# TCGGroup/Torch_Detection

Hardware: AMD Instinct MI355X
Metric: images/sec ResNet-50-FPN fwd+bwd 1333x800 (higher is better)
Workload: dtype bf16; 1 GPU; ResNet-50 + FPN(256, 5 levels) forward+backward, 2 x 3x800x1344 (1333x800 zero-padded to /32) per GPU, BN eval (reference default), fixed cotangents, all parameter grads; global_batch=2, parallelism=dp1, weights_static=True

## Files before the change

### include/tdn.h

```cpp
#ifndef TDN_H_
#define TDN_H_

#include <stddef.h>
#include <stdint.h>

#ifdef __cplusplus
extern "C" {
#endif

#define TDN_VERSION 100

enum { TDN_BF16 = 0, TDN_F16 = 1 };

enum {
  TDN_ADD_NONE = 0,
  TDN_ADD_SAME = 1,
  TDN_ADD_UP2X = 2,
  TDN_ADD_SUMPOOL2 = 3
};

typedef struct tdn_epilogue {
  const float* scale;
  const float* shift;
  const void* addend;
// ... 30 lines not shown

int64_t tdn_conv2d_wgrad_workspace(int N, int H, int W, int Cin, int Cout, int k, int stride,
                                    int pad);

int tdn_conv2d_wgrad(const void* x, const void* g, const void* w_fwd, const float* scale,
                     const float* mean, const float* invstd, float* dw, float* dgamma,
                     float* dbeta, float beta, int N, int H, int W, int Cin, int Cout, int k,
                     int stride, int pad, void* workspace, int64_t workspace_bytes, int dtype,
                     void* stream);

enum { TDN_WGRAD_CONV = 0, TDN_WGRAD_STEM = 1, TDN_WGRAD_GCONV = 2 };
typedef struct tdn_wgrad_item {
  const void* x;
  const void* g;
  const void* w_fwd;
  const float* scale;
  const float* mean;
  const float* invstd;
  float* dw;
  float* dgamma;
  float* dbeta;
  float beta;
  int32_t kind;
  int32_t N, H, W;
  int32_t Cin, Cout;
  int32_t k, stride, pad;
  int32_t groups;
  int32_t reserved;
} tdn_wgrad_item;
int64_t tdn_wgrad_group_workspace(const tdn_wgrad_item* items, int n, int dtype);
int tdn_wgrad_group(const tdn_wgrad_item* items, int n, void* workspace, int64_t workspace_bytes, int dtype,
                    void* stream);
int tdn_wgrad_group_plan(const tdn_wgrad_item* items, int n, int dtype, int32_t* per_item, int32_t* totals);

typedef struct tdn_prep_item {
  const float* w;
  void* w_fwd;
  void* w_dgrad;
  const float* gamma;
  const float* beta;
  const float* mean;
  const float* var;
  float* fold;
  int64_t s_o, s_i, s_h, s_w;
  int32_t Cout, Cin, kh, kw;
  float eps;
  int32_t reserved;
} tdn_prep_item;
int tdn_prepare_group(const tdn_prep_item* items, int n, int dtype, void* stream);

typedef struct tdn_bottleneck_args {
  const void* in;
  const void* w1;
  const void* w2;
  const void* w3;
  const float* scale1; const float* shift1;
  const float* scale2; const float* shift2;
  const float* scale3; const float* shift3;
  const void* mask1;
  const void* mask2;
  const void* mask3;
  void* out1;
  void* out2;
  void* out3;
  int32_t N, H, W, C;
  void* bits1;
// ... 300 lines not shown
```

### torch_detection_amd/_lib.py

```python
import ctypes
import os
import threading

import torch

_HERE = os.path.dirname(os.path.abspath(__file__))
LIB_PATH = os.path.join(_HERE, os.path.basename(os.environ.get("TDN_LIB", "") or "libtdn.so"))

TDN_BF16 = 0
TDN_F16 = 1
TDN_F32 = 2
NMS_SEG_MAX = 4096
RPN_MAX_LEVELS = 8
RPN_MAX_NUM = 8192
ROI_MAX_LEVELS = 8
ROI_MAX_OUT = 16
ROI_MAX_SAMPLES = 512
TARGET_MAX_GT = 256
TARGET_MAX_BOXES = 1 << 20
TARGET_MAX_NUM = 8192
LOSS_MAX_LEVELS = 8
LOSS_MAX_CLASSES = 1024
LOSS_MAX_ROWS = 1 << 20
LOSS_MAX_AVG = 64
# ... 132 lines not shown
                ("scale3", c_void_p), ("shift3", c_void_p),
                ("mask1", c_void_p), ("mask2", c_void_p), ("mask3", c_void_p),
                ("out1", c_void_p), ("out2", c_void_p), ("out3", c_void_p),
                ("N", ctypes.c_int32), ("H", ctypes.c_int32), ("W", ctypes.c_int32), ("C", ctypes.c_int32),
                ("bits1", c_void_p), ("bits2", c_void_p), ("bits3", c_void_p)]


_BA = ctypes.POINTER(BottleneckArgs)


class BottleneckHeadArgs(ctypes.Structure):
    _fields_ = [("b", BottleneckArgs), ("addend", c_void_p), ("wd", c_void_p), ("scale_d", c_void_p),
                ("shift_d", c_void_p)]


_BHA = ctypes.POINTER(BottleneckHeadArgs)

SIGNATURES = {
    "tdn_last_error": (ctypes.c_char_p, []),
    "tdn_version": (c_int, []),
    "tdn_bn_fold": (c_int, [c_void_p] * 4 + [c_float, c_int] + [c_void_p] * 3 + [c_void_p]),
    "tdn_pack_conv_weight": (c_int, [c_void_p, c_i64, c_i64, c_i64, c_i64, c_int, c_int, c_int, c_int,
                                     c_void_p, c_void_p, c_void_p, c_int, c_void_p]),
    "tdn_pack_stem_weight": (c_int, [c_void_p, c_int, c_void_p, c_int, c_void_p]),
    "tdn_prepare_group": (c_int, [_PI, c_int, c_int, c_void_p]),
    "tdn_conv2d_fwd": (c_int, [c_void_p] * 3 + [c_int] * 8 + [_EP, c_int, c_void_p]),
    "tdn_conv2d_dgrad": (c_int, [c_void_p] * 3 + [c_int] * 8 + [_EP, c_int, c_void_p]),
    "tdn_conv2d_wgrad_workspace": (c_i64, [c_int] * 8),
    "tdn_conv2d_wgrad": (c_int, [c_void_p] * 9 + [c_float] + [c_int] * 8 + [c_void_p, c_i64, c_int, c_void_p]),
    "tdn_wgrad_group_workspace": (c_i64, [_WI, c_int, c_int]),
    "tdn_wgrad_group": (c_int, [_WI, c_int, c_void_p, c_i64, c_int, c_void_p]),
    "tdn_wgrad_group_plan": (c_int, [_WI, c_int, c_int, ctypes.POINTER(ctypes.c_int32),
                                     ctypes.POINTER(ctypes.c_int32)]),
    "tdn_stage_image": (c_int, [c_void_p, c_i64, c_i64, c_i64, c_i64, c_int, c_int, c_int, c_void_p, c_int,
                                c_void_p]),
    "tdn_stem_conv_fwd": (c_int, [c_void_p] * 3 + [c_int] * 4 + [_EP, c_int, c_void_p]),
    "tdn_stem_pool_fwd": (c_int, [c_void_p] * 6 + [c_int] * 5 + [c_void_p]),
    "tdn_stem_conv_wgrad_workspace": (c_i64, [c_int] * 4),
    "tdn_stem_conv_wgrad": (c_int, [c_void_p] * 9 + [c_float] + [c_int] * 4 + [c_void_p, c_i64, c_int, c_void_p]),
    "tdn_maxpool3x3s2_fwd": (c_int, [c_void_p] * 3 + [c_int] * 5 + [c_void_p]),
    "tdn_maxpool3x3s2_bwd": (c_int, [c_void_p] * 4 + [c_int] * 5 + [c_void_p]),
    "tdn_maxpool3x3s2_relu_bwd": (c_int, [c_void_p] * 4 + [c_int] * 5 + [c_void_p]),
    "tdn_subsample2_fwd": (c_int, [c_void_p] * 2 + [c_int] * 5 + [c_void_p]),
    "tdn_subsample2_bwd": (c_int, [c_void_p] * 3 + [c_int] * 5 + [c_void_p]),
    "tdn_add_relu_mask": (c_int, [c_void_p] * 4 + [c_i64, c_int, c_void_p]),
    "tdn_clamp_max": (c_int, [c_void_p, c_float, c_i64, c_int, c_void_p]),
    "tdn_act_mask": (c_int, [c_void_p] * 3 + [c_float, c_i64, c_int, c_void_p]),
    "tdn_channel_affine_fwd": (c_int, [c_void_p] * 4 + [c_i64, c_int, c_int, c_int, c_void_p]),
    "tdn_channel_affine_bwd_workspace": (c_i64, [c_i64, c_int]),
    "tdn_channel_affine_bwd": (c_int, [c_void_p] * 8 + [c_float, c_i64, c_int, c_void_p, c_i64, c_int, c_void_p]),
    "tdn_nchw_f32_to_nhwc": (c_int, [c_void_p, c_i64, c_i64, c_i64, c_i64, c_int, c_int, c_int, c_int, c_void_p,
                                     c_int, c_void_p]),
    "tdn_nchw16_to_nhwc": (c_int, [c_void_p, c_i64, c_i64, c_i64, c_i64, c_int, c_int, c_int, c_int, c_void_p,
                                   c_void_p]),
    "tdn_nhwc_to_nchw_f32": (c_int, [c_void_p, c_int, c_int, c_int, c_int, c_void_p, c_int, c_void_p]),
    "tdn_anchor_grid": (c_int, [c_void_p, c_int, c_int, c_int, c_int, c_int, c_int, c_void_p, c_void_p, c_void_p]),
    "tdn_anchor_pyramid": (c_int, [_AL, c_int, c_void_p, c_void_p, c_void_p]),
    "tdn_bbox_iou_pairwise": (c_int, [c_void_p, c_int, c_void_p, c_int, c_void_p, c_void_p]),
    "tdn_nms_workspace": (c_i64, [c_int]),
    "tdn_nms": (c_int, [c_void_p, c_void_p, c_int, c_float, c_void_p, c_void_p, c_void_p, c_void_p, c_i64,
                        c_void_p]),
    "tdn_bbox_normalize": (c_int, [c_void_p, c_i64, ctypes.POINTER(c_float), ctypes.POINTER(c_float), c_void_p]),
    "tdn_bbox_denormalize": (c_int, [c_void_p, c_void_p, c_i64, c_int, ctypes.POINTER(c_float),
                                     ctypes.POINTER(c_float), c_void_p]),
    "tdn_bbox2delta": (c_int, [c_void_p, c_void_p, c_i64, ctypes.POINTER(c_float), ctypes.POINTER(c_float), c_void_p,
                               c_void_p]),
# ... 123 lines not shown
```

### torch_detection_amd/csrc/conv_wgrad.hip

```cpp
#include "conv_host.h"
#include <limits.h>
#include <string.h>
#include <type_traits>
#include <algorithm>
#include <math.h>
#include <mutex>
#include <unordered_map>
#include <vector>

constexpr int WG_MAXI = 26;
constexpr int FIN_MAXI = 30;

struct WgItem {
  const bf16_t* x;
  const bf16_t* g;
  const bf16_t* w_fwd;
  const float* scale;
  float* out;
  float* colsum;
  float* dotpart;
  int Hin, Win, Cpix, Ktap;
  int Ho, Wo, Cout, sa;
  int M, Mchunk, splitk;
  int ntaps, Ktot;
  int tiles_co, tiles_k;
  int tapgen;
  int grouped;
  int direct;
  float beta;
  int reserved;
};

struct WgGroup {
  int nitems, reserved;
  int blk_start[WG_MAXI + 2];
  WgItem it[WG_MAXI];
};
static_assert(sizeof(WgGroup) <= 4096, "kernel-argument block too large");

__device__ __forceinline__ void wg_tap(int tapgen, int t, int& dh, int& dw) {
  const int k = tapgen & 0xff, pad = (tapgen >> 8) & 0xff, dil = (tapgen >> 16) & 0xff;
  if (tapgen >> 24) { dh = t; dw = 0; return; }
  const int kh = t / k, kw = t - kh * k;
  dh = kh * dil - pad;
  dw = kw * dil - pad;
}

__device__ __forceinline__ bool wg_work(int bid, int splitk, int ntiles, int& split, int& tile) {
  if (splitk >= 8) {
    const int xj = bid >> 3;
    split = (bid & 7) + 8 * (xj / ntiles);
    tile = xj - (xj / ntiles) * ntiles;
  } else {
    split = bid / ntiles;
    tile = bid - split * ntiles;
  }
  return split < splitk;
}
static int wg_blocks(int splitk, int ntiles) {
  const int slots = splitk >= 8 ? 8 * ((splitk + 7) / 8) : splitk;
  return (slots * ntiles + 7) & ~7;
}

template <int RB>
__device__ __forceinline__ int tr_swz(int row) {
  if constexpr (RB >= 256) return (row & 3) | (((row >> 3) & 1) << 2);
  else if constexpr (RB == 128) return ((row >> 1) & 1) | (((row >> 3) & 1) << 1);
  else return (row >> 3) & 1;
}

template <int N>
__device__ __forceinline__ void wg_wait_vm_and_barrier() {
  asm volatile("s_waitcnt vmcnt(%0)\n\ts_barrier" ::"n"(N) : "memory");
}

#ifdef TDN_TRACE_BUILD
__device__ unsigned long long* g_wg_trace = nullptr;
__device__ int g_wg_trace_cap = 0;
#define WG_STAMP(slot, val)                                                                        \
  do {                                                                                             \
    if (g_wg_trace && tid == 0 && (int)blockIdx.x < g_wg_trace_cap)                                \
      g_wg_trace[(size_t)blockIdx.x * 8 + (slot)] = (unsigned long long)(val);                     \
  } while (0)
extern "C" int tdn_debug_wgrad_trace(void* buf, int nwg_cap) {
  unsigned long long* b = (unsigned long long*)buf;
  hipError_t e = hipMemcpyToSymbol(HIP_SYMBOL(g_wg_trace), &b, sizeof(b));
  TDN_CHECK(e == hipSuccess, "tdn_debug_wgrad_trace: %s", hipGetErrorString(e));
  e = hipMemcpyToSymbol(HIP_SYMBOL(g_wg_trace_cap), &nwg_cap, sizeof(nwg_cap));
  TDN_CHECK(e == hipSuccess, "tdn_debug_wgrad_trace: %s", hipGetErrorString(e));
  return 0;
}
#else
#define WG_STAMP(slot, val) do { } while (0)
#endif

template <int BMW , int BNW , int WM, int WN, int NST, bool F16>
__global__ __launch_bounds__(WM * WN * 64) void conv_wgrad_group_kernel(const WgGroup grp) {
  extern __shared__ __attribute__((aligned(16))) char smem[];
  constexpr int BKW = 64;
  constexpr int RBG = BMW * 2, RBX = BNW * 2;
  constexpr int G_BYTES = BKW * RBG, X_BYTES = BKW * RBX, STAGE = G_BYTES + X_BYTES;
  constexpr int RPIG = 1024 / RBG, RPIX = 1024 / RBX;
  constexpr int NW = WM * WN;
  constexpr int G_IT = BKW / (RPIG * NW), X_IT = BKW / (RPIX * NW);
  static_assert(G_IT >= 1 && X_IT >= 1, "every wave must issue the same number of loads per stage (counted vmcnt)");
  constexpr int LOADS = G_IT + X_IT;
  static_assert(LOADS * (NST - 2) < 64, "vmcnt immediate out of range");
  constexpr int WTM = BMW / WM, WTN = BNW / WN, FM = WTM / 16, FN = WTN / 16;
  static_assert(FM >= 1 && FN >= 1, "tile too small");
  static_assert((RPIG * NW) % 16 == 0 && (RPIX * NW) % 16 == 0, "loader round must be a multiple of 16 rows");
  static_assert(WN * BMW * 4 <= NST * STAGE, "cross-wave reduction buffer must fit the ring");

  const int tid = threadIdx.x;
  const int lane = tid & 63;
  const int wave = __builtin_amdgcn_readfirstlane(tid >> 6);

  int idx = 0;
#pragma unroll
  for (int i = 1; i < WG_MAXI; ++i) idx += ((int)blockIdx.x >= grp.blk_start[i]) ? 1 : 0;
  const WgItem& p = grp.it[idx];
  const int ntiles = p.tiles_co * p.tiles_k;
  int split, tile;
  if (!wg_work((int)blockIdx.x - grp.blk_start[idx], p.splitk, ntiles, split, tile)) return;
  WG_STAMP(0, __builtin_readcyclecounter());
  WG_STAMP(4, __builtin_amdgcn_s_memrealtime());
  const int tile_co = tile % p.tiles_co, tile_k = tile / p.tiles_co;
  const int co0 = tile_co * BMW;
  const int kt_per_tap = p.Ktap / BNW;
  const int tap_i = tile_k / kt_per_tap;
  const int ci_k = (tile_k - tap_i * kt_per_tap) * BNW;
  const int ci0 = p.grouped ? co0 : ci_k;
  int dh, dw;
  wg_tap(p.tapgen, tap_i, dh, dw);
  const int m_begin = split * p.Mchunk;
  const int m_end = min(p.M, m_begin + p.Mchunk);
  const int Cout = p.Cout, Cpix = p.Cpix, Hin = p.Hin, Win = p.Win, sa = p.sa, Wo = p.Wo, Ho = p.Ho;
  const bf16_t* const gx = p.x;
  const bf16_t* const gg = p.g;

  constexpr int CPRG = RBG / 16, CPRX = RBX / 16;
  const int g_lrow = lane / CPRG, g_pc = lane % CPRG;
  const int x_lrow = lane / CPRX, x_pc = lane % CPRX;
  const int g_row0 = wave * RPIG + g_lrow;
  const int x_row0 = wave * RPIX + x_lrow;
  const int g_src_el = ((((g_pc >> 1) ^ tr_swz<RBG>(g_row0)) << 1) | (g_pc & 1)) * 8;
  const int x_src_el = ((((x_pc >> 1) ^ tr_swz<RBX>(x_row0)) << 1) | (x_pc & 1)) * 8;
  const bf16_t* zero = (const bf16_t*)g_zero_page;

  int xa[X_IT], xb[X_IT], ximg[X_IT];
  const int HoWo = Ho * Wo;
#pragma unroll
  for (int it = 0; it < X_IT; ++it) {
    const int m = m_begin + it * (RPIX * NW) + x_row0;
    const int img = m / HoWo;
    const int rem = m - img * HoWo;
    ximg[it] = img;
// ... 157 lines not shown
      float d = dpart[i];
      d += __shfl_xor(d, 16, 64);
      d += __shfl_xor(d, 32, 64);
      if (grp4 == 0) red[wn * BMW + wm * WTM + i * 16 + fr] = d;
    }
    __syncthreads();
    for (int c = tid; c < BMW; c += NW * 64) {
      float s = red[c];
#pragma unroll
      for (int w = 1; w < WN; ++w) s += red[w * BMW + c];
      p.dotpart[(int64_t)tile_k * Cout + co0 + c] = s;
    }
  }
}

template <bool F16, int WMR = 4>
__global__ __launch_bounds__(WMR * 128) void conv_wgrad9_group_kernel(const WgGroup grp) {
  extern __shared__ __attribute__((aligned(16))) char smem[];
  constexpr int BKW = 64, BMW = 32 * WMR, BNW = 64;
  constexpr int NWV = WMR * 2;
  constexpr int RBG = BMW * 2, RBX = BNW * 2;
  constexpr int CPRG = RBG / 16, RPIG = 64 / CPRG;
  constexpr int XIT = 64 / (NWV * 8);
  static_assert(RPIG * NWV == 32 && XIT >= 1, "loader layout");
  constexpr int G_TILE = BKW * RBG;
  constexpr int XROWS = 72;
  constexpr int X_TILE = XROWS * RBX;
  constexpr int STAGE = G_TILE + 3 * X_TILE;
  constexpr int FM = 2, FN = 2, WN = 2, WTM = 16 * FM, WTN = 16 * FN;
  const int tid = threadIdx.x;
  const int lane = tid & 63;
  const int wave = __builtin_amdgcn_readfirstlane(tid >> 6);

  int idx = 0;
#pragma unroll
  for (int i = 1; i < WG_MAXI; ++i) idx += ((int)blockIdx.x >= grp.blk_start[i]) ? 1 : 0;
  const WgItem& p = grp.it[idx];
  const int ntiles = p.tiles_co * p.tiles_k;
  int split, tile;
  if (!wg_work((int)blockIdx.x - grp.blk_start[idx], p.splitk, ntiles, split, tile)) return;
  const int tile_co = tile % p.tiles_co, tile_ci = tile / p.tiles_co;
  const int co0 = tile_co * BMW, ci0 = tile_ci * BNW;
  const int m_begin = split * p.Mchunk;
  const int pM = p.M;
  const int m_end = min(pM, m_begin + p.Mchunk);
  const int W = p.Wo, H = p.Ho;
  const int Cout = p.Cout, Cpix = p.Cpix;
  const bf16_t* const gx = p.x;
  const bf16_t* const gg = p.g;
  const bf16_t* zero = (const bf16_t*)g_zero_page;

  const int g_lrow = lane / CPRG, g_pc = lane % CPRG;
  const int x_lrow = lane >> 3, x_pc = lane & 7;
  const int g_row0 = wave * RPIG + g_lrow;
  const int x_row0 = wave * 8 + x_lrow;
  const int g_src_el = ((((g_pc >> 1) ^ tr_swz<RBG>(g_row0)) << 1) | (g_pc & 1)) * 8;
  const int x_src_el = ((((x_pc >> 1) ^ tr_swz<RBX>(x_row0)) << 1) | (x_pc & 1)) * 8;
  int xh[XIT + 1], xw[XIT + 1];
#pragma unroll
  for (int it = 0; it <= XIT; ++it) {
    const int q = m_begin + it * (NWV * 8) + x_row0 - 1;
    const int qq = q < 0 ? q + W * H : q;
    xw[it] = qq % W;
    xh[it] = (qq / W) % H;
  }

  auto stage_load = [&](int mt, int s) {
    char* sG = smem + s * STAGE;
    char* sX = sG + G_TILE;
#pragma unroll
    for (int it = 0; it < 2; ++it) {
      const int m = mt + it * 32 + g_row0;
      const bf16_t* src = (m < m_end) ? gg + ((int64_t)m * Cout + co0 + g_src_el) : zero + (g_src_el & 127);
// ... 329 lines not shown
    if (tid == 0) {
      const float d = (red[0] + red[1]) + (red[2] + red[3]);
      if (p.dbeta) p.dbeta[co] = (beta != 0.f) ? beta * p.dbeta[co] + cs : cs;
      if (p.mean && p.invstd && p.dgamma) {
        const float dg = (d - p.mean[co] * cs) * p.invstd[co];
        p.dgamma[co] = (beta != 0.f) ? beta * p.dgamma[co] + dg : dg;
      }
    }
  }
}

#define TDN_TAP_SHAPES(X) \
  X(0, 64, 32, 2, 2, 2, 6, 1800)      \
  X(1, 64, 64, 2, 2, 2, 5, 2000)                            \
  X(2, 64, 64, 2, 2, 3, 3, 1365)                            \
  X(3, 128, 64, 2, 2, 2, 3, 2050)                           \
  X(4, 128, 64, 2, 2, 3, 2, 1640)                           \
  X(5, 256, 64, 4, 2, 2, 2, 2000)                           \
  X(6, 256, 64, 4, 2, 3, 1, 1460)                           \
  X(7, 128, 128, 2, 2, 2, 2, 2180)                          \
  X(8, 256, 128, 4, 2, 2, 1, 1750)
struct TapShape { int bmw, bnw, wm, wn, nst, per_cu, step_clk; };
#define TDN_TAP_ROW(id, bmw, bnw, wm, wn, nst, per_cu, step_clk) {bmw, bnw, wm, wn, nst, per_cu, step_clk},
static const TapShape kTapShapes[] = {TDN_TAP_SHAPES(TDN_TAP_ROW)};
static const int kNumTapShapes = (int)(sizeof(kTapShapes) / sizeof(kTapShapes[0]));
static const int kT9StepClk = 2600;

struct ItemPlan {
  int Hin, Win, Cpix, Ktap, Ho, Wo, Cout, sa, M, ntaps, Ktot, tapgen, grouped, map_mode;
  bool t9_ok, bn;
  int variant;
  int shape;
  int tiles_co, tiles_k, splitk, mchunk, direct, blocks, ndot;
  int step_clk, tmin, slots;
  int64_t off_out, off_colsum, off_dot;
};

static int item_geometry(const tdn_wgrad_item& it, ItemPlan& g) {
  TDN_CHECK(it.x && it.g && it.w_fwd && it.dw, "wgrad item: NULL pointer");
  TDN_CHECK(it.N > 0 && it.H > 0 && it.W > 0, "wgrad item: bad tensor shape N=%d H=%d W=%d", it.N, it.H, it.W);
  g.grouped = 0;
  g.t9_ok = false;
  g.bn = it.mean && it.invstd && it.dgamma;
  if (it.kind == TDN_WGRAD_STEM) {
    TDN_CHECK(it.H % 2 == 0 && it.W % 2 == 0 && it.Cout % 64 == 0, "stem wgrad: bad shape");
    g.Hin = it.H + 6; g.Win = it.W + 8; g.Cpix = 4; g.Ktap = 32; g.Ho = it.H / 2; g.Wo = it.W / 2;
    g.Cout = it.Cout; g.sa = 2; g.ntaps = 7; g.tapgen = 1 << 24; g.map_mode = 1;
  } else {
    TDN_CHECK(it.kind == TDN_WGRAD_CONV || it.kind == TDN_WGRAD_GCONV, "wgrad item: bad kind %d", it.kind);
    const int k = it.k, stride = it.stride, pad = it.pad;
    if (conv_check_rules(k, stride, pad, it.Cin, it.Cout)) return -1;
    g.Hin = it.H; g.Win = it.W; g.Cpix = it.Cin; g.Ktap = it.Cin;
    g.Ho = conv_out_sz(it.H, k, stride, pad); g.Wo = conv_out_sz(it.W, k, stride, pad);
    g.Cout = it.Cout; g.sa = stride; g.ntaps = k * k;
    g.tapgen = k | (pad << 8) | (conv_dil(k, pad) << 16);
    g.map_mode = 0;
    if (it.kind == TDN_WGRAD_GCONV) {
      const int C = it.Cout, groups = it.groups;
      TDN_CHECK(it.Cin == it.Cout, "grouped conv: Cin must equal Cout");
      TDN_CHECK(groups > 0 && C % groups == 0 && C % 64 == 0 && (C / groups) <= 64 && 64 % (C / groups) == 0,
                "grouped conv: need C %% 64 == 0 and channels per group dividing 64 (C=%d, groups=%d)", C, groups);
      g.grouped = 1; g.Ktap = 64; g.map_mode = 4 * (C / groups);
    } else {
      g.t9_ok = (k == 3 && stride == 1 && pad == 1 && it.W >= 8 && it.Cout % 64 == 0 && it.Cin % 64 == 0);
    }
  }
  TDN_CHECK(g.Ho > 0 && g.Wo > 0, "wgrad item: empty output");
  TDN_CHECK((int64_t)it.N * g.Ho * g.Wo < (1ll << 31) / 4 && (int64_t)it.N * g.Hin * g.Win < (1ll << 31) / 4,
            "tensor too large for 32-bit pixel indexing");
  g.M = it.N * g.Ho * g.Wo;
  g.Ktot = g.ntaps * g.Ktap;
  return 0;
}

static std::mutex g_plan_mutex;
static std::unordered_map<uint64_t, double> g_plan_cache;

static inline int launch_key(const ItemPlan& g) { return g.variant ? -g.variant : g.shape; }

static void launch_lists(const std::vector<ItemPlan>& plans, std::vector<std::vector<int>>& lists) {
  const int n = (int)plans.size();
  for (int key = -2; key < kNumTapShapes; ++key) {
    std::vector<int> cur;
    for (int i = 0; i < n; ++i) {
      if (launch_key(plans[i]) != key) continue;
      cur.push_back(i);
      if ((int)cur.size() == WG_MAXI) { lists.push_back(cur); cur.clear(); }
    }
    if (!cur.empty()) lists.push_back(cur);
  }
}

static void split_member(ItemPlan& g, int T) {
  const int ksteps = ceil_div(g.M, 64);
  if (T < 1) T = 1;
  int splitk = (ksteps + T / 2) / T;
  if (splitk < 1) splitk = 1;
  if (splitk > 256) splitk = 256;
  if (splitk >= 8) splitk = (splitk + 4) / 8 * 8;
  const int mchunk = ceil_div(ceil_div(g.M, splitk), 64) * 64;
  g.splitk = ceil_div(g.M, mchunk);
  g.mchunk = mchunk;
  g.blocks = wg_blocks(g.splitk, g.tiles_co * g.tiles_k);
}

static double model_group(const std::vector<ItemPlan>& plans, const std::vector<std::vector<int>>& lists) {
  double total = 0.0, slab_bytes = 0.0;
  std::vector<double> heap;
  for (const std::vector<int>& L : lists) {
    const int slots = plans[L[0]].slots;
    heap.assign(slots, 0.0);
    auto cmp = [](double a, double b) { return a > b; };
    double end = 0.0;
    for (int i : L) {
      const ItemPlan& g = plans[i];
      const int tile_floats = g.variant ? 9 * (g.variant == 2 ? 64 : 128) * 64 : kTapShapes[g.shape].bmw * kTapShapes[g.shape].bnw;
      const double c = (double)ceil_div(g.mchunk, 64) * g.step_clk + tile_floats * 4.0 / 20.0 + 3000.0;
      const int live = g.splitk * g.tiles_co * g.tiles_k;
      for (int b = 0; b < live; ++b) {
        std::pop_heap(heap.begin(), heap.end(), cmp);
        const double t = heap.back() + c;
        heap.back() = t;
        std::push_heap(heap.begin(), heap.end(), cmp);
        if (t > end) end = t;
      }
      if (!g.direct) slab_bytes += (double)g.splitk * g.Cout * g.Ktot * 4.0;
    }
    total += end;
  }
  return total + slab_bytes / 4096.0;
}

static int plan_group(const tdn_wgrad_item* items, int n, std::vector<ItemPlan>& plans, int64_t* ws_floats) {
  TDN_CHECK(items != nullptr && n > 0, "wgrad group: no items");
  plans.resize(n);
  const int t9_mode = tdn_knob_int("TDN_WGRAD9", 1);
  const int t9_64 = tdn_knob_int("TDN_WGRAD9_64", 1);
  const int shape_env = tdn_knob_int("TDN_WGRAD_SHAPE", -1);
  const int s256 = tdn_knob_int("TDN_WGRAD_S256", 8), s128 = tdn_knob_int("TDN_WGRAD_S128", 4), s64 = tdn_knob_int("TDN_WGRAD_S64", 2);
  const int s256f = tdn_knob_int("TDN_WGRAD_S256F", 5);
  const int uniform = tdn_knob_int("TDN_WGRAD_UNIFORM", 0);
  const int tmin_tap = tdn_knob_int("TDN_WGRAD_TMIN", 24), tmin_t9 = tdn_knob_int("TDN_WGRAD9_TMIN", 32);
  const int direct_ok = tdn_knob_int("TDN_WGRAD_DIRECT", 1);
  int min_bmw = 256;
  for (int i = 0; i < n; ++i) {
    ItemPlan& g = plans[i];
    if (item_geometry(items[i], g)) return -1;
    g.variant = (g.t9_ok && t9_mode != 0) ? (g.Cout % 128 == 0 ? 1 : (t9_64 ? 2 : 0)) : 0;
    if (!g.variant && !g.grouped && g.Ktap != 32) {
      const int b = g.Cout % 256 == 0 ? 256 : (g.Cout % 128 == 0 ? 128 : 64);
      if (b < min_bmw) min_bmw = b;
    }
  }
  for (int i = 0; i < n; ++i) {
    ItemPlan& g = plans[i];
    if (g.variant) {
      g.shape = -1;
      g.tiles_co = g.Cout / (g.variant == 2 ? 64 : 128);
      g.tiles_k = g.Ktap / 64;
      g.step_clk = kT9StepClk;
      g.tmin = tmin_t9;
      g.slots = g.variant == 2 ? 512 : 256;
    } else {
      int bmw = g.Cout % 256 == 0 ? 256 : (g.Cout % 128 == 0 ? 128 : 64);
      if (uniform && bmw > min_bmw) bmw = min_bmw;
      int shape = g.Ktap == 32 ? 0 : ((g.grouped || bmw == 64) ? s64 : (bmw == 128 ? s128 : s256));
      auto fits = [&](int sh) {
        return sh >= 0 && sh < kNumTapShapes && g.Cout % kTapShapes[sh].bmw == 0 && g.Ktap % kTapShapes[sh].bnw == 0 &&
               !(g.grouped && (kTapShapes[sh].bmw != 64 || kTapShapes[sh].bnw != 64));
      };
      if (!fits(shape) && bmw == 256 && !g.grouped && fits(s256f)) shape = s256f;
      if (!fits(shape)) shape = g.Ktap == 32 ? 0 : (g.Ktap % 64 == 0 ? 2 : 0);
      if (shape_env >= 0 && shape_env < kNumTapShapes && !g.grouped && g.Cout % kTapShapes[shape_env].bmw == 0 &&
          g.Ktap % kTapShapes[shape_env].bnw == 0)
        shape = shape_env;
      g.shape = shape;
      const TapShape& s = kTapShapes[shape];
      g.tiles_co = g.Cout / s.bmw;
      g.tiles_k = g.ntaps * (g.Ktap / s.bnw);
      g.step_clk = s.step_clk;
      g.tmin = tmin_tap;
      g.slots = 256 * s.per_cu;
    }
  }
  std::vector<std::vector<int>> lists;
  launch_lists(plans, lists);
  const double dmin = tdn_knob_int("TDN_WGRAD_DMIN", 40000), dmax = tdn_knob_int("TDN_WGRAD_DMAX", 400000);
  const int fixed_t = tdn_knob_int("TDN_WGRAD_T", 0);
  uint64_t key = 1469598103934665603ull;
  auto mix = [&key](int64_t v) { key = (key ^ (uint64_t)v) * 1099511628211ull; };
  mix(n); mix((int64_t)dmin); mix((int64_t)dmax); mix(fixed_t);
  for (const ItemPlan& g : plans) {
    mix(g.M); mix(g.Cout); mix(g.Ktap); mix(g.ntaps); mix(g.variant); mix(g.shape); mix(g.tmin); mix(g.map_mode);
    mix(g.step_clk);
  }
  double best = -1.0, bestD = dmin;
  bool hit = false;
  {
    std::lock_guard<std::mutex> lock(g_plan_mutex);
    auto itc = g_plan_cache.find(key);
    if (itc != g_plan_cache.end()) { bestD = itc->second; hit = true; }
  }
  const int ncand = (fixed_t > 0 || hit) ? 0 : 24;
  for (int c = 0; c < ncand; ++c) {
    const double D = dmin * pow(dmax / dmin, ncand > 1 ? (double)c / (ncand - 1) : 0.0);
    for (ItemPlan& g : plans) {
      int T = fixed_t > 0 ? fixed_t : (int)(D / g.step_clk + 0.5);
      if (T < g.tmin) T = g.tmin;
      split_member(g, T);
      g.direct = (g.splitk == 1 && g.map_mode == 0 && direct_ok) ? 1 : 0;
    }
    const double t = model_group(plans, lists);
    if (best < 0 || t < best) { best = t; bestD = D; }
  }
  if (ncand > 0) {
    std::lock_guard<std::mutex> lock(g_plan_mutex);
    g_plan_cache[key] = bestD;
  }
  int64_t off = 0;
  for (int i = 0; i < n; ++i) {
    ItemPlan& g = plans[i];
    int T = fixed_t > 0 ? fixed_t : (int)(bestD / g.step_clk + 0.5);
    if (T < g.tmin) T = g.tmin;
    split_member(g, T);
    g.direct = (g.splitk == 1 && g.map_mode == 0 && direct_ok) ? 1 : 0;
    g.ndot = (g.direct && g.bn) ? g.tiles_k : 0;
    g.off_out = off;
    if (!g.direct) off += (int64_t)g.splitk * g.Cout * g.Ktot;
    g.off_colsum = off;
    off += (int64_t)g.splitk * g.Cout;
    g.off_dot = off;
    off += (int64_t)g.ndot * g.Cout;
    off = (off + 63) & ~(int64_t)63;
  }
  *ws_floats = off;
  return 0;
}

template <int BMW, int BNW, int WM, int WN, int NST, bool F16>
static int launch_tap_t(const WgGroup& grp, int nblocks, hipStream_t stream) {
  constexpr size_t lds = (size_t)NST * 64 * (BMW + BNW) * 2;
  if (tdn_allow_lds<conv_wgrad_group_kernel<BMW, BNW, WM, WN, NST, F16>>((int)lds, "conv_wgrad_group") < 0) return -1;
  TDN_LAUNCH((conv_wgrad_group_kernel<BMW, BNW, WM, WN, NST, F16>), dim3(nblocks), dim3(WM * WN * 64), lds,
                     stream, grp);
  TDN_LAUNCH_CHECK();
  return 0;
}

template <bool F16>
static int launch_tap(int shape, const WgGroup& grp, int nblocks, hipStream_t stream) {
#define TDN_TAP_CASE(id, bmw, bnw, wm, wn, nst, per_cu, step_clk) \
  case id: return launch_tap_t<bmw, bnw, wm, wn, nst, F16>(grp, nblocks, stream);
  switch (shape) {
    TDN_TAP_SHAPES(TDN_TAP_CASE)
    default: tdn_set_error("wgrad: bad tile shape id %d", shape); return -1;
  }
}

template <bool F16, int WMR>
static int launch_t9(const WgGroup& grp, int nblocks, hipStream_t stream) {
  constexpr size_t lds = 2 * (size_t)(64 * (64 * WMR) + 3 * 72 * 128);
  if (tdn_allow_lds<conv_wgrad9_group_kernel<F16, WMR>>((int)lds, "conv_wgrad9_group") < 0) return -1;
  TDN_LAUNCH((conv_wgrad9_group_kernel<F16, WMR>), dim3(nblocks), dim3(WMR * 128), lds, stream, grp);
  TDN_LAUNCH_CHECK();
  return 0;
}

static void fill_item(WgItem& d, const tdn_wgrad_item& it, const ItemPlan& g, float* ws) {
  memset(&d, 0, sizeof(d));
  d.x = (const bf16_t*)it.x; d.g = (const bf16_t*)it.g; d.w_fwd = (const bf16_t*)it.w_fwd;
  d.scale = it.scale;
  d.out = g.direct ? it.dw : ws + g.off_out;
  d.colsum = ws + g.off_colsum;
  d.dotpart = g.ndot ? ws + g.off_dot : nullptr;
  d.Hin = g.Hin; d.Win = g.Win; d.Cpix = g.Cpix; d.Ktap = g.Ktap; d.Ho = g.Ho; d.Wo = g.Wo; d.Cout = g.Cout;
  d.sa = g.sa; d.M = g.M; d.Mchunk = g.mchunk; d.splitk = g.splitk; d.ntaps = g.ntaps; d.Ktot = g.Ktot;
  d.tiles_co = g.tiles_co; d.tiles_k = g.tiles_k; d.tapgen = g.tapgen; d.grouped = g.grouped; d.direct = g.direct;
  d.beta = it.beta;
}

extern "C" int64_t tdn_wgrad_group_workspace(const tdn_wgrad_item* items, int n, int dtype) {
  TDN_CHECK_DTYPE(dtype);
  std::vector<ItemPlan> plans;
  int64_t fl = 0;
  if (plan_group(items, n, plans, &fl)) return -1;
  return fl * 4 + 256;
}

extern "C" int tdn_wgrad_group_plan(const tdn_wgrad_item* items, int n, int dtype, int32_t* per_item,
                                    int32_t* totals) {
  TDN_CHECK_DTYPE(dtype);
  std::vector<ItemPlan> plans;
  int64_t fl = 0;
  if (plan_group(items, n, plans, &fl)) return -1;
  std::vector<std::vector<int>> lists;
  launch_lists(plans, lists);
  int64_t blocks = 0, slab_kib = 0;
  for (int i = 0; i < n; ++i) {
    const ItemPlan& g = plans[i];
    const int64_t slab = g.direct ? 0 : (int64_t)g.splitk * g.Cout * g.Ktot * 4 / 1024;
    if (per_item) {
      int32_t* o = per_item + 8 * i;
      o[0] = g.variant; o[1] = g.variant ? (g.variant == 2 ? 64 : 128) : kTapShapes[g.shape].bmw; o[2] = g.variant ? 64 : kTapShapes[g.shape].bnw;
      o[3] = g.splitk; o[4] = g.mchunk; o[5] = g.direct; o[6] = g.blocks; o[7] = (int32_t)slab;
    }
    blocks += g.blocks;
    slab_kib += slab;
  }
  if (totals) {
    totals[0] = (int32_t)lists.size();
    totals[1] = ceil_div(n, FIN_MAXI);
    totals[2] = (int32_t)blocks;
    totals[3] = (int32_t)slab_kib;
  }
  return 0;
}

extern "C" int tdn_wgrad_group(const tdn_wgrad_item* items, int n, void* workspace, int64_t workspace_bytes,
                               int dtype, void* stream_) {
  TDN_CHECK_DTYPE(dtype);
  hipStream_t stream = (hipStream_t)stream_;
  std::vector<ItemPlan> plans;
  int64_t fl = 0;
  if (plan_group(items, n, plans, &fl)) return -1;
  TDN_CHECK(workspace != nullptr && workspace_bytes >= fl * 4, "wgrad workspace too small: %lld < %lld",
            (long long)workspace_bytes, (long long)(fl * 4));
  TDN_CHECK(((uintptr_t)workspace & 15) == 0, "wgrad workspace must be 16-byte aligned");
  float* ws = (float*)workspace;
  std::vector<std::vector<int>> lists;
  launch_lists(plans, lists);
  for (const std::vector<int>& L : lists) {
    WgGroup grp;
    memset(&grp, 0, sizeof(grp));
    grp.nitems = (int)L.size();
    grp.reserved = tdn_knob_int("TDN_WGRAD9_STAGGER", 1);
    int blk = 0;
    for (int j = 0; j < WG_MAXI + 2; ++j) grp.blk_start[j] = INT_MAX;
    for (int j = 0; j < (int)L.size(); ++j) {
      const int i = L[j];
      grp.blk_start[j] = blk;
      fill_item(grp.it[j], items[i], plans[i], ws);
      blk += plans[i].blocks;
    }
    const ItemPlan& g0 = plans[L[0]];
    int rc;
    if (g0.variant == 2) rc = dtype == TDN_F16 ? launch_t9<true, 2>(grp, blk, stream) : launch_t9<false, 2>(grp, blk, stream);
    else if (g0.variant) rc = dtype == TDN_F16 ? launch_t9<true, 4>(grp, blk, stream) : launch_t9<false, 4>(grp, blk, stream);
    else rc = dtype == TDN_F16 ? launch_tap<true>(g0.shape, grp, blk, stream) : launch_tap<false>(g0.shape, grp, blk, stream);
    if (rc) return rc;
  }
  for (int base = 0; base < n; base += FIN_MAXI) {
    FinGroup fg;
    memset(&fg, 0, sizeof(fg));
    const int cnt = (n - base < FIN_MAXI) ? n - base : FIN_MAXI;
    fg.nitems = cnt;
    for (int j = 0; j < FIN_MAXI + 2; ++j) fg.blk_start[j] = INT_MAX;
    int blk = 0;
    for (int j = 0; j < cnt; ++j) {
      const tdn_wgrad_item& it = items[base + j];
      const ItemPlan& g = plans[base + j];
      FinItem& f = fg.it[j];
      fg.blk_start[j] = blk;
      f.slab = g.direct ? nullptr : ws + g.off_out;
      f.colsum = ws + g.off_colsum;
      f.dotpart = g.ndot ? ws + g.off_dot : nullptr;
      f.w_fwd = (const bf16_t*)it.w_fwd;
      f.scale = it.scale; f.mean = it.mean; f.invstd = it.invstd;
      f.dw = it.dw; f.dgamma = it.dgamma; f.dbeta = it.dbeta; f.beta = it.beta;
      f.splitk = g.splitk; f.Cout = g.Cout; f.Ktot = g.Ktot; f.map_mode = g.map_mode; f.ndot = g.ndot;
      int k4p = 1;
      while (k4p < (g.Ktot >> 2) && k4p < 256) k4p <<= 1;
      f.K4P = k4p;
      blk += g.direct ? ceil_div(g.Cout, 256) : g.Cout;
    }
    if (dtype == TDN_F16)
      TDN_LAUNCH(wgrad_finalize_group_kernel<true>, dim3(blk), dim3(256), 0, stream, fg);
// ... 85 lines not shown
```

Baseline: 533.2 images/sec.

## Balance grouped wgrad blocks across XCDs with per-XCD queue map

Adds a host-built work map for the grouped weight-gradient launch. Low-split items are pooled, split into tile segments, and greedily assigned to eight per-XCD queues by estimated cost, with block index mod 8 selecting the queue. The aim is to even out load across XCDs and reduce the tail. It also adds a tile-order swap for tall items and caches the maps in the plan memo. The price is a more complex per-block index decode in the kernel and more planning work on cache misses.

New measurement: 533.1 images/sec. About the same (-0.0%).

```diff
diff --git a/include/tdn.h b/include/tdn.h
--- a/include/tdn.h
+++ b/include/tdn.h
@@ -86,6 +86,7 @@
 int tdn_wgrad_group(const tdn_wgrad_item* items, int n, void* workspace, int64_t workspace_bytes, int dtype,
                     void* stream);
 int tdn_wgrad_group_plan(const tdn_wgrad_item* items, int n, int dtype, int32_t* per_item, int32_t* totals);
+int tdn_wgrad_group_map(const tdn_wgrad_item* items, int n, int dtype, int32_t* out, int64_t cap);
 
 typedef struct tdn_prep_item {
   const float* w;
diff --git a/torch_detection_amd/_lib.py b/torch_detection_amd/_lib.py
--- a/torch_detection_amd/_lib.py
+++ b/torch_detection_amd/_lib.py
@@ -188,6 +188,7 @@
     "tdn_wgrad_group": (c_int, [_WI, c_int, c_void_p, c_i64, c_int, c_void_p]),
     "tdn_wgrad_group_plan": (c_int, [_WI, c_int, c_int, ctypes.POINTER(ctypes.c_int32),
                                      ctypes.POINTER(ctypes.c_int32)]),
+    "tdn_wgrad_group_map": (c_int, [_WI, c_int, c_int, ctypes.POINTER(ctypes.c_int32), c_i64]),
     "tdn_stage_image": (c_int, [c_void_p, c_i64, c_i64, c_i64, c_i64, c_int, c_int, c_int, c_void_p, c_int,
                                 c_void_p]),
     "tdn_stem_conv_fwd": (c_int, [c_void_p] * 3 + [c_int] * 4 + [_EP, c_int, c_void_p]),
diff --git a/torch_detection_amd/csrc/conv_wgrad.hip b/torch_detection_amd/csrc/conv_wgrad.hip
--- a/torch_detection_amd/csrc/conv_wgrad.hip
+++ b/torch_detection_amd/csrc/conv_wgrad.hip
@@ -28,12 +28,23 @@
   int grouped;
   int direct;
   float beta;
-  int reserved;
+  int tile_order;
+};
+
+constexpr int WG_MAXSEG = 80;
+struct WgMap {
+  int grid;
+  int pool_start, pool_blocks;
+  int blk_start[WG_MAXI + 2];
+  unsigned short qlen[8];
+  unsigned char xcd_first[12];
+  unsigned seg_qt[WG_MAXSEG];
+  unsigned char seg_ms[WG_MAXSEG];
 };
 
 struct WgGroup {
   int nitems, reserved;
-  int blk_start[WG_MAXI + 2];
+  WgMap map;
   WgItem it[WG_MAXI];
 };
 static_assert(sizeof(WgGroup) <= 4096, "kernel-argument block too large");
@@ -46,8 +57,31 @@
   dw = kw * dil - pad;
 }
 
-__device__ __forceinline__ bool wg_work(int bid, int splitk, int ntiles, int& split, int& tile) {
-  if (splitk >= 8) {
+__host__ __device__ __forceinline__ bool wg_work(const WgGroup& grp, int b, int& idx, int& split, int& tile) {
+  const WgMap& m = grp.map;
+  const int pb = b - m.pool_start;
+  if (pb >= 0 && pb < m.pool_blocks) {
+    const int x = pb & 7, q = pb >> 3;
+    if (q >= (int)m.qlen[x]) return false;
+    const int s = m.xcd_first[x], e = m.xcd_first[x + 1];
+    int k = s;
+    for (int j = s + 1; j < e; ++j) k += ((int)(m.seg_qt[j] >> 16) <= q) ? 1 : 0;
+    const unsigned qt = m.seg_qt[k];
+    const int ms = m.seg_ms[k];
+    idx = ms >> 3;
+    split = ms & 7;
+    const WgItem& p = grp.it[idx];
+    const int t = (int)(qt & 0xffffu) + q - (int)(qt >> 16);
+    tile = p.tile_order ? (t % p.tiles_k) * p.tiles_co + t / p.tiles_k : t;
+    return true;
+  }
+  const int bid0 = pb < 0 ? b : pb - m.pool_blocks;
+  idx = 0;
+#pragma unroll
+  for (int i = 1; i < WG_MAXI; ++i) idx += (bid0 >= m.blk_start[i]) ? 1 : 0;
+  const WgItem& p = grp.it[idx];
+  const int bid = bid0 - m.blk_start[idx], ntiles = p.tiles_co * p.tiles_k;
+  if (p.splitk >= 8) {
     const int xj = bid >> 3;
     split = (bid & 7) + 8 * (xj / ntiles);
     tile = xj - (xj / ntiles) * ntiles;
@@ -55,7 +89,7 @@
     split = bid / ntiles;
     tile = bid - split * ntiles;
   }
-  return split < splitk;
+  return split < p.splitk;
 }
 static int wg_blocks(int splitk, int ntiles) {
   const int slots = splitk >= 8 ? 8 * ((splitk + 7) / 8) : splitk;
@@ -115,13 +149,9 @@
   const int lane = tid & 63;
   const int wave = __builtin_amdgcn_readfirstlane(tid >> 6);
 
-  int idx = 0;
-#pragma unroll
-  for (int i = 1; i < WG_MAXI; ++i) idx += ((int)blockIdx.x >= grp.blk_start[i]) ? 1 : 0;
+  int idx, split, tile;
+  if (!wg_work(grp, (int)blockIdx.x, idx, split, tile)) return;
   const WgItem& p = grp.it[idx];
-  const int ntiles = p.tiles_co * p.tiles_k;
-  int split, tile;
-  if (!wg_work((int)blockIdx.x - grp.blk_start[idx], p.splitk, ntiles, split, tile)) return;
   WG_STAMP(0, __builtin_readcyclecounter());
   WG_STAMP(4, __builtin_amdgcn_s_memrealtime());
   const int tile_co = tile % p.tiles_co, tile_k = tile / p.tiles_co;
@@ -345,13 +375,9 @@
   const int lane = tid & 63;
   const int wave = __builtin_amdgcn_readfirstlane(tid >> 6);
 
-  int idx = 0;
-#pragma unroll
-  for (int i = 1; i < WG_MAXI; ++i) idx += ((int)blockIdx.x >= grp.blk_start[i]) ? 1 : 0;
+  int idx, split, tile;
+  if (!wg_work(grp, (int)blockIdx.x, idx, split, tile)) return;
   const WgItem& p = grp.it[idx];
-  const int ntiles = p.tiles_co * p.tiles_k;
-  int split, tile;
-  if (!wg_work((int)blockIdx.x - grp.blk_start[idx], p.splitk, ntiles, split, tile)) return;
   const int tile_co = tile % p.tiles_co, tile_ci = tile / p.tiles_co;
   const int co0 = tile_co * BMW, ci0 = tile_ci * BNW;
   const int m_begin = split * p.Mchunk;
@@ -747,6 +773,7 @@
   int variant;
   int shape;
   int tiles_co, tiles_k, splitk, mchunk, direct, blocks, ndot;
+  int tile_order;
   int step_clk, tmin, slots;
   int64_t off_out, off_colsum, off_dot;
 };
@@ -789,7 +816,8 @@
 }
 
 static std::mutex g_plan_mutex;
-static std::unordered_map<uint64_t, double> g_plan_cache;
+struct PlanMemo { double D; std::vector<WgMap> maps; };
+static std::unordered_map<uint64_t, PlanMemo> g_plan_cache;
 
 static inline int launch_key(const ItemPlan& g) { return g.variant ? -g.variant : g.shape; }
 
@@ -817,36 +845,177 @@
   g.splitk = ceil_div(g.M, mchunk);
   g.mchunk = mchunk;
   g.blocks = wg_blocks(g.splitk, g.tiles_co * g.tiles_k);
-}
-
-static double model_group(const std::vector<ItemPlan>& plans, const std::vector<std::vector<int>>& lists) {
+  g.tile_order = (g.splitk < 8 && g.Cout > g.Ktot) ? 1 : 0;
+}
+
+static double wg_cost(const ItemPlan& g) {
+  const int tile_floats = g.variant ? 9 * (g.variant == 2 ? 64 : 128) * 64 : kTapShapes[g.shape].bmw * kTapShapes[g.shape].bnw;
+  return (double)ceil_div(g.mchunk, 64) * g.step_clk + tile_floats * 4.0 / 20.0 + 3000.0;
+}
+
+static int wg_build_map(const std::vector<ItemPlan>& plans, const std::vector<int>& L, WgMap& m, bool pool = true) {
+  memset(&m, 0, sizeof(m));
+  for (int j = 0; j < WG_MAXI + 2; ++j) m.blk_start[j] = INT_MAX;
+  const int nL = (int)L.size();
+  std::vector<char> pooled(nL, 0);
+  struct Seg { int j, split, t0, cnt; double cost; };
+  std::vector<Seg> subs;
+  const int S = std::max(1, plans[L[0]].slots / 8);
+  if (pool && tdn_knob_int("TDN_WGRAD_XCDMAP", 1) != 0) {
+    int64_t W = 0;
+    for (int j = 0; j < nL; ++j) {
+      const ItemPlan& g = plans[L[j]];
+      if (g.splitk < 8 && g.tiles_co * g.tiles_k < 65536) W += (int64_t)g.splitk * g.tiles_co * g.tiles_k;
+    }
+    const int64_t Lq = (W + 7) / 8;
+    const int cap = (int)std::min<int64_t>(S, std::max<int64_t>(Lq, 1));
+    int nseg = 0;
+    for (int j = 0; j < nL && Lq < 65536; ++j) {
+      const ItemPlan& g = plans[L[j]];
+      const int ntiles = g.tiles_co * g.tiles_k;
+      if (g.splitk >= 8 || ntiles >= 65536) continue;
+      int k = 1;
+      while (k < 8 && ceil_div(ntiles, k) > cap) k *= 2;
+      if (k > ntiles) k = ntiles;
+      if (nseg + g.splitk * k > WG_MAXSEG - 16) continue;
+      nseg += g.splitk * k;
+      pooled[j] = 1;
+      const int minor = g.tile_order ? g.tiles_k : g.tiles_co, major = ntiles / minor;
+      const double c = wg_cost(g);
+      for (int sp = 0; sp < g.splitk; ++sp)
+        for (int i = 0; i < k; ++i) {
+          const int t0 = major >= k ? (major * i / k) * minor : ntiles * i / k;
+          const int t1 = major >= k ? (major * (i + 1) / k) * minor : ntiles * (i + 1) / k;
+          subs.push_back({j, sp, t0, t1 - t0, c * (t1 - t0)});
+        }
+    }
+  }
+  std::vector<Seg> queue[8];
+  if (!subs.empty()) {
+    std::stable_sort(subs.begin(), subs.end(), [](const Seg& a, const Seg& b) {
+      const double ca = a.cost / a.cnt, cb = b.cost / b.cnt;
+      return ca != cb ? ca > cb : a.cnt > b.cnt;
+    });
+    int W = 0;
+    for (const Seg& u : subs) W += u.cnt;
+    const int G = (W + 7) & ~7, Lr = G / 8;
+    auto cmp = [](double a, double b) { return a > b; };
+    std::vector<double> slot[8], trial;
+    double end[8] = {0}, load[8] = {0};
+    int room[8];
+    for (int x = 0; x < 8; ++x) {
+      room[x] = x < 8 - (G - W) ? Lr : Lr - 1;
+      slot[x].assign(S, 0.0);
+    }
+    auto run = [&](std::vector<double>& h, double e, int cnt, double c) {
+      for (int i = 0; i < cnt; ++i) {
+        std::pop_heap(h.begin(), h.end(), cmp);
+        h.back() += c;
+        if (h.back() > e) e = h.back();
+        std::push_heap(h.begin(), h.end(), cmp);
+      }
+      return e;
+    };
+    for (Seg u : subs) {
+      const double c = u.cost / u.cnt;
+      while (u.cnt > 0) {
+        int x = -1, mv = u.cnt;
+        double best = 0.0;
+        for (int y = 0; y < 8; ++y) {
+          if (room[y] < u.cnt) continue;
+          trial = slot[y];
+          const double e = run(trial, end[y], u.cnt, c);
+          if (x < 0 || e < best || (e == best && load[y] < load[x])) { x = y; best = e; }
+        }
+        if (x < 0) {
+          x = 0;
+          for (int y = 1; y < 8; ++y) if (room[y] > room[x]) x = y;
+          mv = room[x];
+        }
+        queue[x].push_back({u.j, u.split, u.t0, mv, c * mv});
+        end[x] = run(slot[x], end[x], mv, c);
+        load[x] += c * mv;
+        room[x] -= mv;
+        u.t0 += mv; u.cnt -= mv;
+      }
+    }
+    int nseg = 0;
+    for (int x = 0; x < 8; ++x) nseg += (int)queue[x].size();
+    if (nseg > WG_MAXSEG) return wg_build_map(plans, L, m, false);
+    nseg = 0;
+    for (int x = 0; x < 8; ++x) {
+      m.xcd_first[x] = (unsigned char)nseg;
+      int q = 0;
+      for (const Seg& u : queue[x]) {
+        m.seg_qt[nseg] = ((unsigned)q << 16) | (unsigned)u.t0;
+        m.seg_ms[nseg] = (unsigned char)(u.j << 3 | u.split);
+        q += u.cnt;
+        ++nseg;
+      }
+      m.qlen[x] = (unsigned short)q;
+    }
+    for (int x = 8; x < 12; ++x) m.xcd_first[x] = (unsigned char)nseg;
+    m.pool_blocks = G;
+  }
+  int blk = 0;
+  double cost_own = 0.0, cost_pool = 0.0;
+  for (int j = 0; j < nL; ++j) {
+    const double c = wg_cost(plans[L[j]]);
+    if (pooled[j]) { cost_pool = std::max(cost_pool, c); continue; }
+    cost_own = std::max(cost_own, c);
+    m.blk_start[j] = blk;
+    blk += plans[L[j]].blocks;
+  }
+  m.pool_start = cost_own >= cost_pool ? blk : 0;
+  for (int j = nL - 1, next = INT_MAX; j >= 0; --j) {
+    if (pooled[j]) m.blk_start[j] = next;
+    else next = m.blk_start[j];
+  }
+  m.grid = m.pool_blocks + blk;
+  return m.grid;
+}
+
+static void fill_item_map(WgItem& d, const ItemPlan& g) {
+  d.splitk = g.splitk; d.tiles_co = g.tiles_co; d.tiles_k = g.tiles_k; d.tile_order = g.tile_order;
+}
+
+static double model_group(const std::vector<ItemPlan>& plans, const std::vector<std::vector<int>>& lists, bool queues) {
   double total = 0.0, slab_bytes = 0.0;
   std::vector<double> heap;
+  WgGroup grp;
+  memset(&grp, 0, sizeof(grp));
+  const int nq = queues ? 8 : 1;
   for (const std::vector<int>& L : lists) {
-    const int slots = plans[L[0]].slots;
-    heap.assign(slots, 0.0);
+    const int slots = std::max(1, plans[L[0]].slots / nq);
+    const int grid = wg_build_map(plans, L, grp.map, queues);
+    double cost[WG_MAXI];
+    for (int j = 0; j < (int)L.size(); ++j) {
+      const ItemPlan& g = plans[L[j]];
+      fill_item_map(grp.it[j], g);
+      cost[j] = wg_cost(g);
+      if (!g.direct) slab_bytes += (double)g.splitk * g.Cout * g.Ktot * 4.0;
+    }
     auto cmp = [](double a, double b) { return a > b; };
     double end = 0.0;
-    for (int i : L) {
-      const ItemPlan& g = plans[i];
-      const int tile_floats = g.variant ? 9 * (g.variant == 2 ? 64 : 128) * 64 : kTapShapes[g.shape].bmw * kTapShapes[g.shape].bnw;
-      const double c = (double)ceil_div(g.mchunk, 64) * g.step_clk + tile_floats * 4.0 / 20.0 + 3000.0;
-      const int live = g.splitk * g.tiles_co * g.tiles_k;
-      for (int b = 0; b < live; ++b) {
+    for (int x = 0; x < nq; ++x) {
+      heap.assign(slots, 0.0);
+      for (int b = x; b < grid; b += nq) {
+        int idx, split, tile;
+        if (!wg_work(grp, b, idx, split, tile)) continue;
         std::pop_heap(heap.begin(), heap.end(), cmp);
-        const double t = heap.back() + c;
+        const double t = heap.back() + cost[idx];
         heap.back() = t;
         std::push_heap(heap.begin(), heap.end(), cmp);
         if (t > end) end = t;
       }
-      if (!g.direct) slab_bytes += (double)g.splitk * g.Cout * g.Ktot * 4.0;
     }
     total += end;
   }
   return total + slab_bytes / 4096.0;
 }
 
-static int plan_group(const tdn_wgrad_item* items, int n, std::vector<ItemPlan>& plans, int64_t* ws_floats) {
+static int plan_group(const tdn_wgrad_item* items, int n, std::vector<ItemPlan>& plans, int64_t* ws_floats,
+                      std::vector<std::vector<int>>* lists_out = nullptr, std::vector<WgMap>* maps_out = nullptr) {
   TDN_CHECK(items != nullptr && n > 0, "wgrad group: no items");
   plans.resize(n);
   const int t9_mode = tdn_knob_int("TDN_WGRAD9", 1);
@@ -857,6 +1026,7 @@
   const int uniform = tdn_knob_int("TDN_WGRAD_UNIFORM", 0);
   const int tmin_tap = tdn_knob_int("TDN_WGRAD_TMIN", 24), tmin_t9 = tdn_knob_int("TDN_WGRAD9_TMIN", 32);
   const int direct_ok = tdn_knob_int("TDN_WGRAD_DIRECT", 1);
+  const int qmodel = tdn_knob_int("TDN_WGRAD_QMODEL", 0);
   int min_bmw = 256;
   for (int i = 0; i < n; ++i) {
     ItemPlan& g = plans[i];
@@ -904,17 +1074,18 @@
   const int fixed_t = tdn_knob_int("TDN_WGRAD_T", 0);
   uint64_t key = 1469598103934665603ull;
   auto mix = [&key](int64_t v) { key = (key ^ (uint64_t)v) * 1099511628211ull; };
-  mix(n); mix((int64_t)dmin); mix((int64_t)dmax); mix(fixed_t);
+  mix(n); mix((int64_t)dmin); mix((int64_t)dmax); mix(fixed_t); mix(direct_ok); mix(tdn_knob_int("TDN_WGRAD_XCDMAP", 1)); mix(qmodel);
   for (const ItemPlan& g : plans) {
     mix(g.M); mix(g.Cout); mix(g.Ktap); mix(g.ntaps); mix(g.variant); mix(g.shape); mix(g.tmin); mix(g.map_mode);
     mix(g.step_clk);
   }
   double best = -1.0, bestD = dmin;
   bool hit = false;
+  std::vector<WgMap> maps;
   {
     std::lock_guard<std::mutex> lock(g_plan_mutex);
     auto itc = g_plan_cache.find(key);
-    if (itc != g_plan_cache.end()) { bestD = itc->second; hit = true; }
+    if (itc != g_plan_cache.end()) { bestD = itc->second.D; maps = itc->second.maps; hit = true; }
   }
   const int ncand = (fixed_t > 0 || hit) ? 0 : 24;
   for (int c = 0; c < ncand; ++c) {
@@ -925,12 +1096,8 @@
       split_member(g, T);
       g.direct = (g.splitk == 1 && g.map_mode == 0 && direct_ok) ? 1 : 0;
     }
-    const double t = model_group(plans, lists);
+    const double t = model_group(plans, lists, qmodel != 0);
     if (best < 0 || t < best) { best = t; bestD = D; }
-  }
-  if (ncand > 0) {
-    std::lock_guard<std::mutex> lock(g_plan_mutex);
-    g_plan_cache[key] = bestD;
   }
   int64_t off = 0;
   for (int i = 0; i < n; ++i) {
@@ -949,6 +1116,14 @@
     off = (off + 63) & ~(int64_t)63;
   }
   *ws_floats = off;
+  if (!hit) {
+    maps.resize(lists.size());
+    for (size_t li = 0; li < lists.size(); ++li) wg_build_map(plans, lists[li], maps[li]);
+    std::lock_guard<std::mutex> lock(g_plan_mutex);
+    g_plan_cache[key] = PlanMemo{bestD, maps};
+  }
+  if (lists_out) lists_out->swap(lists);
+  if (maps_out) maps_out->swap(maps);
   return 0;
 }
 
@@ -992,6 +1167,7 @@
   d.sa = g.sa; d.M = g.M; d.Mchunk = g.mchunk; d.splitk = g.splitk; d.ntaps = g.ntaps; d.Ktot = g.Ktot;
   d.tiles_co = g.tiles_co; d.tiles_k = g.tiles_k; d.tapgen = g.tapgen; d.grouped = g.grouped; d.direct = g.direct;
   d.beta = it.beta;
+  d.tile_order = g.tile_order;
 }
 
 extern "C" int64_t tdn_wgrad_group_workspace(const tdn_wgrad_item* items, int n, int dtype) {
@@ -1007,10 +1183,11 @@
   TDN_CHECK_DTYPE(dtype);
   std::vector<ItemPlan> plans;
   int64_t fl = 0;
-  if (plan_group(items, n, plans, &fl)) return -1;
   std::vector<std::vector<int>> lists;
-  launch_lists(plans, lists);
+  std::vector<WgMap> maps;
+  if (plan_group(items, n, plans, &fl, &lists, &maps)) return -1;
   int64_t blocks = 0, slab_kib = 0;
+  for (const WgMap& m : maps) blocks += m.grid;
   for (int i = 0; i < n; ++i) {
     const ItemPlan& g = plans[i];
     const int64_t slab = g.direct ? 0 : (int64_t)g.splitk * g.Cout * g.Ktot * 4 / 1024;
@@ -1019,7 +1196,6 @@
       o[0] = g.variant; o[1] = g.variant ? (g.variant == 2 ? 64 : 128) : kTapShapes[g.shape].bmw; o[2] = g.variant ? 64 : kTapShapes[g.shape].bnw;
       o[3] = g.splitk; o[4] = g.mchunk; o[5] = g.direct; o[6] = g.blocks; o[7] = (int32_t)slab;
     }
-    blocks += g.blocks;
     slab_kib += slab;
   }
   if (totals) {
@@ -1031,32 +1207,56 @@
   return 0;
 }
 
+extern "C" int tdn_wgrad_group_map(const tdn_wgrad_item* items, int n, int dtype, int32_t* out, int64_t cap) {
+  TDN_CHECK_DTYPE(dtype);
+  std::vector<ItemPlan> plans;
+  std::vector<std::vector<int>> lists;
+  std::vector<WgMap> maps;
+  int64_t fl = 0;
+  if (plan_group(items, n, plans, &fl, &lists, &maps)) return -1;
+  int64_t rows = 0;
+  WgGroup grp;
+  for (size_t li = 0; li < lists.size(); ++li) {
+    const std::vector<int>& L = lists[li];
+    memset(&grp, 0, sizeof(grp));
+    grp.map = maps[li];
+    for (int j = 0; j < (int)L.size(); ++j) fill_item_map(grp.it[j], plans[L[j]]);
+    for (int b = 0; b < grp.map.grid; ++b, ++rows) {
+      if (!out || rows >= cap) continue;
+      int idx, split, tile;
+      const bool live = wg_work(grp, b, idx, split, tile);
+      int32_t* o = out + 6 * rows;
+      o[0] = (int32_t)li; o[1] = b;
+      o[2] = live ? L[idx] : -1; o[3] = live ? split : -1; o[4] = live ? tile : -1;
+      o[5] = (b >= grp.map.pool_start && b < grp.map.pool_start + grp.map.pool_blocks) ? 1 : 0;
+    }
+  }
+  TDN_CHECK(rows < (1ll << 31), "wgrad map: too many workgroups");
+  return (int)rows;
+}
+
 extern "C" int tdn_wgrad_group(const tdn_wgrad_item* items, int n, void* workspace, int64_t workspace_bytes,
                                int dtype, void* stream_) {
   TDN_CHECK_DTYPE(dtype);
   hipStream_t stream = (hipStream_t)stream_;
   std::vector<ItemPlan> plans;
+  std::vector<std::vector<int>> lists;
+  std::vector<WgMap> maps;
   int64_t fl = 0;
-  if (plan_group(items, n, plans, &fl)) return -1;
+  if (plan_group(items, n, plans, &fl, &lists, &maps)) return -1;
   TDN_CHECK(workspace != nullptr && workspace_bytes >= fl * 4, "wgrad workspace too small: %lld < %lld",
             (long long)workspace_bytes, (long long)(fl * 4));
   TDN_CHECK(((uintptr_t)workspace & 15) == 0, "wgrad workspace must be 16-byte aligned");
   float* ws = (float*)workspace;
-  std::vector<std::vector<int>> lists;
-  launch_lists(plans, lists);
-  for (const std::vector<int>& L : lists) {
+  for (size_t li = 0; li < lists.size(); ++li) {
+    const std::vector<int>& L = lists[li];
     WgGroup grp;
     memset(&grp, 0, sizeof(grp));
     grp.nitems = (int)L.size();
     grp.reserved = tdn_knob_int("TDN_WGRAD9_STAGGER", 1);
-    int blk = 0;
-    for (int j = 0; j < WG_MAXI + 2; ++j) grp.blk_start[j] = INT_MAX;
-    for (int j = 0; j < (int)L.size(); ++j) {
-      const int i = L[j];
-      grp.blk_start[j] = blk;
-      fill_item(grp.it[j], items[i], plans[i], ws);
-      blk += plans[i].blocks;
-    }
+    grp.map = maps[li];
+    for (int j = 0; j < (int)L.size(); ++j) fill_item(grp.it[j], items[L[j]], plans[L[j]], ws);
+    const int blk = grp.map.grid;
     const ItemPlan& g0 = plans[L[0]];
     int rc;
     if (g0.variant == 2) rc = dtype == TDN_F16 ? launch_t9<true, 2>(grp, blk, stream) : launch_t9<false, 2>(grp, blk, stream);
```
